# yassine-cherni/mujoco_ros2_simulation

Measured on AMD Instinct MI355X. Metric: env-steps/sec (whole node), 7-DoF arm+lidar scene at 1/2/4/8 MI355X, higher is better.
Workload: dtype f32

## Files before the change

### include/mrs.h

```cpp
#ifndef MRS_H
#define MRS_H

#include "mrs_model.h"

#ifdef __cplusplus
extern "C" {
#endif

typedef struct mrs_model mrs_model;
typedef struct mrs_batch mrs_batch;

enum {
  MRS_OK = 0,
  MRS_ERR_INVALID = -1,
  MRS_ERR_LOAD = -2,
  MRS_ERR_DEVICE = -3,
  MRS_ERR_UNSUPPORTED = -4
};

enum {
  MRS_FIELD_QPOS = 0,
  MRS_FIELD_QVEL = 1,
  MRS_FIELD_CTRL = 2,
  MRS_FIELD_QFRC_APPLIED = 3,
// ... 103 lines not shown
int mrs_batch_get_contact_wrench(mrs_batch* b, double* host, int env0, int n);
enum {
  MRS_DYNOUT_QFRC_BIAS = 0,
  MRS_DYNOUT_MASS_MATRIX = 1,
  MRS_DYNOUT_SITE_JAC = 2,
  MRS_DYNOUT_SITE_POSE = 3,
  MRS_DYNOUT_COUNT = 4
};
#define MRS_MAX_JAC_SITES 16
int mrs_batch_set_jac_sites(mrs_batch* b, const int* site_ids, int n);
int mrs_batch_dyn_dim(const mrs_batch* b, int which);
float* mrs_batch_dyn_device_ptr(mrs_batch* b, int which);
int mrs_batch_get_dyn(mrs_batch* b, int which, double* host, int env0, int n);
int mrs_batch_get_efc(mrs_batch* b, int env, int max, int* type, double* J, double* R, double* aref,
                      double* force);
int mrs_batch_get_field_device(mrs_batch* b, int field, float* d_out, int env0, int n);
int mrs_batch_sync(mrs_batch* b);
double mrs_batch_last_kernel_ms(mrs_batch* b, int kind);
int mrs_batch_set_timing(mrs_batch* b, int mask);
int mrs_debug_phase_cycles(double* out, int n, int reset);
int mrs_debug_batch_layout(const mrs_batch* b, int* out, int n);
int mrs_debug_pairs(const mrs_model* m, int* geom, int max, int* pruned);
int mrs_debug_plan_layout(const mrs_model* m, int n_envs, int cu_count, int max_contacts, int* out, int n);
int mrs_debug_render_plan(const mrs_model* m, int cam, int n_frames, int max_lds, long long* out, int n);
int mrs_debug_ray_filter(const mrs_model* m, unsigned group_mask, int flags, int bodyexclude, int* out, int max);

#ifdef __cplusplus
}
#endif
#endif
```

### mujoco_ros2_simulation_amd/csrc/capi.cc

```cpp
#include <algorithm>
#include <cstring>
#include <memory>
#include <stdexcept>
#include <string>
#include <vector>

#include "../../include/mrs.h"
#include "hip/batch.h"
#include "mjcf/model.h"
#include "hip/rayfilter.h"
#include "hip/start_rows.h"
#include "mjcf/xml.h"

struct mrs_model {
  mrs::Model m;
};
struct mrs_batch {
  mrs::BatchImpl* impl = nullptr;
  const mrs_model* model = nullptr;
};

namespace {

thread_local std::string g_last_error;
// ... 542 lines not shown
  return mrs::batch_layout(b->impl, out, n);
}

int mrs_debug_plan_layout(const mrs_model* m, int n_envs, int cu_count, int max_contacts, int* out, int n) {
  int k = 0;
  const int rc = guarded([&] {
    if (!m || !out || n < 0) throw std::invalid_argument("null model or output");
    if (n_envs < 1) throw std::invalid_argument("n_envs must be positive");
    k = mrs::plan_layout(m->m, n_envs, cu_count, max_contacts, out, n);
  });
  return rc == MRS_OK ? k : rc;
}

int mrs_debug_pairs(const mrs_model* m, int* geom, int max, int* pruned) {
  int k = 0;
  const int rc = guarded([&] {
    if (!m) throw std::invalid_argument("null model");
    if (max < 0 || (max > 0 && !geom)) throw std::invalid_argument("null output or negative capacity");
    k = mrs::walked_pairs(m->m, geom, max, pruned);
  });
  return rc == MRS_OK ? k : rc;
}

int mrs_debug_render_plan(const mrs_model* m, int cam, int n_frames, int max_lds, long long* out, int n) {
  int k = 0;
  const int rc = guarded([&] {
    if (!m || !out || n < 0) throw std::invalid_argument("null model or output");
    if (n_frames < 1) throw std::invalid_argument("n_frames must be positive");
    if (max_lds < 0) throw std::invalid_argument("negative LDS limit");
    k = mrs::render_plan(m->m, cam, n_frames, max_lds, out, n);
  });
  return rc == MRS_OK ? k : rc;
}

int mrs_debug_ray_filter(const mrs_model* m, unsigned group_mask, int flags, int bodyexclude, int* out, int max) {
  int k = 0;
  const int rc = guarded([&] {
    if (!m) throw std::invalid_argument("null model");
    if (max < 0 || (max > 0 && !out)) throw std::invalid_argument("null output or negative capacity");
    mrs::check_ray_filter(m->m, flags, bodyexclude);
    const std::vector<mrs::RayGeom> list =
        mrs::build_ray_filter(m->m, group_mask, (flags & MRS_RAY_NO_STATIC) != 0, bodyexclude);
    k = static_cast<int>(list.size());
    for (int i = 0; i < k && i < max; ++i) out[i] = list[i].id;
  });
  return rc == MRS_OK ? k : rc;
// ... 4 lines not shown
```

### mujoco_ros2_simulation_amd/csrc/hip/batch.h

```cpp
#pragma once

#include <stdexcept>
#include <string>

namespace mrs {

struct Model;
struct BatchImpl;

struct DeviceError : std::runtime_error { using std::runtime_error::runtime_error; };
struct UnsupportedError : std::runtime_error { using std::runtime_error::runtime_error; };

BatchImpl* batch_create(const Model* model, int n_envs, int device, int max_contacts);
void batch_free(BatchImpl* b);
int batch_num_envs(const BatchImpl* b);
int batch_layout(const BatchImpl* b, int* out, int n);
int plan_layout(const Model& m, int n_envs, int cu_count, int max_contacts, int* out, int n);
int walked_pairs(const Model& m, int* geom, int max, int* pruned);
void batch_set_stream(BatchImpl* b, void* stream);
void batch_reset(BatchImpl* b, int key, int env0, int n);
void batch_set_start_states(BatchImpl* b, const double* qpos, const double* qvel, int count);
void batch_set_start_states_device(BatchImpl* b, const float* d_qpos, const float* d_qvel, int count);
int batch_num_start_states(const BatchImpl* b);
void batch_reset_masked_device(BatchImpl* b, const unsigned char* d_mask, const int* d_key, int key);
void batch_reset_masked(BatchImpl* b, const unsigned char* mask, const int* keys, int key);
void batch_set(BatchImpl* b, int field, const double* host, int env0, int n);
void batch_get(BatchImpl* b, int field, double* host, int env0, int n);
void* batch_device_ptr(BatchImpl* b, int field);
void batch_set_act(BatchImpl* b, const double* host, int env0, int n);
void batch_get_act(BatchImpl* b, double* host, int env0, int n);
float* batch_act_device_ptr(BatchImpl* b);
void batch_set_mocap(BatchImpl* b, const double* pos, const double* quat, int env0, int n);
void batch_get_mocap(BatchImpl* b, double* pos, double* quat, int env0, int n);
float* batch_mocap_pos_device_ptr(BatchImpl* b);
float* batch_mocap_quat_device_ptr(BatchImpl* b);
int batch_param_dim(BatchImpl* b, int param);
void batch_set_param(BatchImpl* b, int param, const double* host, int env0, int n);
void batch_get_param(BatchImpl* b, int param, double* host, int env0, int n);
float* batch_param_device_ptr(BatchImpl* b, int param);
int batch_inertial_dim(BatchImpl* b, int which);
void batch_set_inertial(BatchImpl* b, const double* mass, const double* inertia, const double* armature, int env0, int n);
// ... 31 lines not shown
```

### mujoco_ros2_simulation_amd/csrc/hip/batch.hip

```cpp
#include <hip/hip_runtime.h>

#include <algorithm>
#include <cmath>
#include <cstdio>
#include <cstdlib>
#include <cstring>
#include <deque>
#include <initializer_list>
#include <stdexcept>
#include <string>
#include <thread>
#include <type_traits>
#include <utility>
#include <vector>

#include "../../../include/mrs.h"
#include "../mjcf/model.h"
#include "batch.h"
#include "batch_impl.h"
#include "devmodel.h"
#include "devtables.h"
#include "plan.h"
#include "lit.h"
#include "start_rows.h"
// ... 147 lines not shown
  for (int id = 0; id < kArrCount; ++id) {
    const EnvArray a = env_array(b, id);
    if (a.made == EnvArray::ON_USE || (a.made == EnvArray::IF_DIM && a.dim == 0)) continue;
    a.bind(dalloc(b, static_cast<size_t>(b.n) * std::max(1, a.dim) * a.width()));
  }
}

void build_devmodel(BatchImpl& b, int max_con_req, const Overrides& o) {
  const Model& m = *b.model;
  const DevTables T = build_tables(m, max_con_req, o);
  int cus = 0;
  if (hipDeviceGetAttribute(&cus, hipDeviceAttributeMultiprocessorCount, b.device) != hipSuccess) cus = 0;
  const Plan p = choose_plan(m, T, b.n, cus, o);
  void* made[kArrCount];
  for (int id = 0; id < kArrCount; ++id) made[id] = env_array(b, id).ptr;
  b.dm = p.dm;
  for (int id = 0; id < kArrCount; ++id)
    if (made[id]) env_array(b, id).bind(made[id]);
  b.dblock_f = dalloc(b, T.f.size() * sizeof(float));
  b.dblock_i = dalloc(b, T.i.size() * sizeof(int));
  HIP_CHECK(hipMemcpyAsync(b.dblock_f, T.f.data(), T.f.size() * sizeof(float), hipMemcpyHostToDevice, b.stream));
  HIP_CHECK(hipMemcpyAsync(b.dblock_i, T.i.data(), T.i.size() * sizeof(int), hipMemcpyHostToDevice, b.stream));
  T.patch(b.dm, static_cast<const float*>(b.dblock_f), static_cast<const int*>(b.dblock_i));
  b.dm.rf_static = b.dm.rf_mode ? static_cast<float*>(dalloc(b, std::max(1, b.dm.nrf) * sizeof(float))) : nullptr;
  b.group = p.group; b.g16_one_wg = p.g16_one_wg; b.wpb16 = p.wpb16; b.helpers = p.helpers; b.ext = p.ext;
  b.pair_g1 = T.pair_g1; b.pair_g2 = T.pair_g2; b.pair_dim = T.pair_dim; b.pair_mu = T.pair_mu;
  b.pairs_pruned = T.pairs_pruned;
  b.d_dm = static_cast<DevModel*>(dalloc(b, sizeof(DevModel)));
  HIP_CHECK(hipMemcpyAsync(b.d_dm, &b.dm, sizeof(DevModel), hipMemcpyHostToDevice, b.stream));
  HIP_CHECK(hipStreamSynchronize(b.stream));
}

struct RowStage { double* host; std::vector<float> f; std::vector<int> i; };

void rows_to_device(BatchImpl& b, int env0, int n, std::initializer_list<std::pair<EnvArray, const double*>> parts) {
  HIP_CHECK(hipSetDevice(b.device));
  std::deque<RowStage> stage;
  bool queued = false;
  for (const auto& part : parts) {
    const EnvArray& a = part.first;
    const double* host = part.second;
    const size_t cnt = static_cast<size_t>(n) * std::max(0, a.dim);
    if (!host || cnt == 0) continue;
    const void* src = host;
    if (a.type == EnvArray::F32) {
      std::vector<float>& t = stage.emplace_back().f;
      t.resize(cnt);
// ... 207 lines not shown
  return b;
}

void batch_free(BatchImpl* b) {
  if (!b) return;
  (void)hipSetDevice(b->device);
  if (b->stream) (void)hipStreamSynchronize(b->stream);
  if (b->rstream) (void)hipStreamSynchronize(b->rstream);
  for (void* p : b->allocs) (void)hipFree(p);
  if (b->pool_qpos) (void)hipFree(b->pool_qpos);
  if (b->pool_qvel) (void)hipFree(b->pool_qvel);
  render_free(*b);
  for (int k = 0; k < 2; ++k) {
    if (b->ev0[k]) (void)hipEventDestroy(b->ev0[k]);
    if (b->ev1[k]) (void)hipEventDestroy(b->ev1[k]);
  }
  if (b->own_stream) (void)hipStreamDestroy(b->own_stream);
  delete b;
}

int batch_num_envs(const BatchImpl* b) { return b->n; }

int batch_layout(const BatchImpl* b, int* out, int n) {
  int v[21];
  plan_layout_values(b->dm, b->group, b->g16_one_wg, b->wpb16, b->helpers, v);
  v[16] = b->dm.cfrc_contact ? 1 : 0;
  v[17] = b->dm.dyn_mask;
  v[18] = b->dm.solve_fuse;
  v[19] = b->dm.npair;
  v[20] = b->pairs_pruned;
  int k = 0;
  for (; k < n && k < 21; ++k) out[k] = v[k];
  return k;
}

int walked_pairs(const Model& m, int* geom, int max, int* pruned) {
  const DevTables T = build_tables(m, 0, read_overrides());
  const int k = static_cast<int>(T.pair_g1.size());
  for (int q = 0; q < k && q < max; ++q) { geom[2 * q] = T.pair_g1[q]; geom[2 * q + 1] = T.pair_g2[q]; }
  if (pruned) *pruned = T.pairs_pruned;
  return k;
}

int plan_layout(const Model& m, int n_envs, int cu_count, int max_contacts, int* out, int n) {
  const Overrides o = read_overrides();
  const DevTables T = build_tables(m, max_contacts, o);
  const Plan p = choose_plan(m, T, n_envs, cu_count, o);
  int v[kPlanLayoutValues];
  plan_layout_values(p.dm, p.group, p.g16_one_wg, p.wpb16, p.helpers, v);
  int k = 0;
  for (; k < n && k < kPlanLayoutValues; ++k) out[k] = v[k];
  return k;
}

void batch_set_stream(BatchImpl* b, void* stream) {
  b->stream = stream ? static_cast<hipStream_t>(stream) : b->own_stream;
}

void batch_reset(BatchImpl* b, int key, int env0, int n) {
  const Model& m = *b->model;
  check_env_range(*b, env0, n);
  if (key >= m.nkey) throw std::invalid_argument("keyframe index out of range");
  b->ctrl_bound = nullptr;
  if (n == 0) return;
// ... 504 lines not shown
```

### mujoco_ros2_simulation_amd/csrc/hip/devmodel.h

```cpp
#pragma once

#include <cstdint>

#include "../../../include/mrs_model.h"

namespace mrs {

#if !defined(__HIPCC__)
#define __device__
#define __forceinline__ inline
#endif
template <class T>
struct CPtr {
  const T* p;
  CPtr& operator=(const T* q) { p = q; return *this; }
  __device__ __forceinline__ T operator[](int i) const {
#if defined(__HIP_DEVICE_COMPILE__)
    return ((const __attribute__((address_space(4))) T*)p)[i];
#else
    return p[i];
#endif
  }
  __device__ __forceinline__ CPtr operator+(int i) const { return CPtr{p + i}; }
};
// ... 119 lines not shown
  CPtr<float> rfray;
  int rf_sweep, rf_sw_n, rf_sw_full, rf_sw_adr0, rf_sw_plo, rf_sw_phi;
  float rf_sw[16];
  const float* xfrc;
  int na;
  int prm_mask;
  CPtr<float> actdyn;
  int nmocap;
  float *mocap_pos, *mocap_quat;
  const float *prm_gain, *prm_bias, *prm_damp, *prm_fric;
  int npair_explicit;
  const float* prm_inr;
  int inr_dim;
  float* cfrc_contact;
  int dyn_mask, dyn_nsel;
  float* dyn_out[4];
  int dyn_site[16];
  int solve_fuse;
  int nten_spatial, lds_tenJ;
  CPtr<int> tsp_ten, tsp_adr, tsp_num, ten_sp;
  CPtr<float> tsp_seg;
  int nact_site, nact_site_vel;
  CPtr<float> sact;
};
constexpr int kRayBlock = 128;
constexpr int kPrmGain = 1, kPrmBias = 2, kPrmDamp = 4, kPrmFric = 8;
constexpr int kPrmInr = 16;
constexpr int kDynBias = 1, kDynM = 2, kDynJac = 4, kDynPose = 8;

template <int G>
#ifndef MRS_G16_WAVES
#define MRS_G16_WAVES 4
#endif
struct WavesPerBlock { static constexpr int value = G == 64 ? 1 : (G == 16 ? MRS_G16_WAVES : 4); };
inline int envs_per_block(int g, int wpb16 = WavesPerBlock<16>::value) {
  switch (g) {
    case 8: return WavesPerBlock<8>::value * 8;
    case 16: return wpb16 * 4;
    case 32: return WavesPerBlock<32>::value * 2;
    default: return WavesPerBlock<64>::value;
  }
}

struct DevState {
  float *qpos, *qvel, *ctrl, *qfrc_applied, *qacc_ws, *qacc, *qfrc_act, *sensordata;
  double* time;
// ... 17 lines not shown
```

### mujoco_ros2_simulation_amd/csrc/hip/devtables.h

```cpp
#pragma once

#include <algorithm>
#include <array>
#include <cmath>
#include <cstdlib>
#include <cstring>
#include <functional>
#include <stdexcept>
#include <string>
#include <vector>

#include "../../../include/mrs.h"
#include "../mjcf/model.h"
#include "batch.h"
#include "devmodel.h"
#include "renderplan.h"
#include "start_rows.h"

namespace mrs {

struct Overrides {
  int group = 0;
  int g16_wpb = 0;
  bool g16_one_wg = false;
  bool ray_helpers = true;
  bool no_fuse_ih = false;
  bool no_solve_fuse = false;
  bool no_ray_sweep = false;
  bool no_pair_prune = false;
  bool no_static_rays = false;
  bool no_static_frame = false;
  bool kin_twopass = false;
  int sparse_off = 0;
  int diag_skip = 0;
  bool sensors_every_step = false;
  bool no_multiccd = false;
  bool no_bvh = false;
  int bvh_leaf = 4;
  bool bvh_median = false;
  int spread = 0;
};

inline Overrides read_overrides() {
  auto set = [](const char* name) { return std::getenv(name) != nullptr; };
  auto num = [](const char* name, int absent) { const char* e = std::getenv(name); return e ? std::atoi(e) : absent; };
  Overrides o;
  o.group = num("MRS_GROUP", 0);
  o.g16_wpb = num("MRS_G16_WPB", 0);
  o.g16_one_wg = set("MRS_G16_ONE_WG");
  o.ray_helpers = num("MRS_RAY_HELPERS", 1) != 0;
  o.no_fuse_ih = set("MRS_NO_FUSE_IH");
  o.no_solve_fuse = set("MRS_NO_SOLVE_FUSE");
  o.no_ray_sweep = set("MRS_NO_RAY_SWEEP");
  o.no_pair_prune = set("MRS_NO_PAIR_PRUNE");
  o.no_static_rays = set("MRS_NO_STATIC_RAYS");
  o.no_static_frame = set("MRS_NO_STATIC_FRAME");
  o.kin_twopass = set("MRS_KIN_TWOPASS");
  o.sparse_off = num("MRS_SPARSE_OFF", 0) & 15;
  o.diag_skip = num("MRS_DIAG_SKIP", 0);
  o.sensors_every_step = num("MRS_SENSORS_EVERY_STEP", 0) != 0;
  o.no_multiccd = set("MRS_NO_MULTICCD");
  o.no_bvh = set("MRS_NO_BVH");
  o.bvh_leaf = std::max(1, std::min(64, num("MRS_BVH_LEAF", 4)));
  o.bvh_median = set("MRS_BVH_MEDIAN");
  o.spread = std::max(0, std::min(3, num("MRS_SPREAD", 0)));
  return o;
}

constexpr int kRlitHead = 12, kRlitLight = 24, kRlitMat = 12, kRlitTex = 16, kRlitMaxLights = 8;

template <class T>
struct Slot {
  CPtr<T> DevModel::*member;
  size_t off, len;
};
// ... 9 lines not shown
  int pairs_pruned = 0;
  bool convex_pairs = false;
  std::vector<int> rf;
  bool rf_fixed = false;

  void addf(CPtr<float> DevModel::*dst, const std::vector<double>& v) {
    fslot.push_back({dst, f.size(), v.size()});
    for (double x : v) f.push_back(static_cast<float>(x));
    while (f.size() % 4) f.push_back(0);
  }
  void addf(CPtr<float> DevModel::*dst, const std::vector<float>& v) {
    fslot.push_back({dst, f.size(), v.size()});
    f.insert(f.end(), v.begin(), v.end());
    while (f.size() % 4) f.push_back(0);
  }
  void addi(CPtr<int> DevModel::*dst, const std::vector<int>& v) {
    islot.push_back({dst, i.size(), v.size()});
    i.insert(i.end(), v.begin(), v.end());
    while (i.size() % 4) i.push_back(0);
  }
  const float* table(CPtr<float> DevModel::*member) const {
    for (const auto& s : fslot)
      if (s.member == member) return f.data() + s.off;
    throw std::logic_error("table not packed");
  }
  void patch(DevModel& d, const float* fbase, const int* ibase) const {
    for (const auto& s : fslot) (d.*s.member).p = fbase + s.off;
    for (const auto& s : islot) (d.*s.member).p = ibase + s.off;
  }
};

inline float int_bits(int v) { float f; std::memcpy(&f, &v, sizeof f); return f; }
inline int bits_int(float f) { int v; std::memcpy(&v, &f, sizeof v); return v; }

inline void quat_to_mat(const double q[4], double R[9]) {
  R[0] = q[0] * q[0] + q[1] * q[1] - q[2] * q[2] - q[3] * q[3]; R[1] = 2 * (q[1] * q[2] - q[0] * q[3]);
  R[2] = 2 * (q[1] * q[3] + q[0] * q[2]); R[3] = 2 * (q[1] * q[2] + q[0] * q[3]);
  R[4] = q[0] * q[0] - q[1] * q[1] + q[2] * q[2] - q[3] * q[3]; R[5] = 2 * (q[2] * q[3] - q[0] * q[1]);
  R[6] = 2 * (q[1] * q[3] - q[0] * q[2]); R[7] = 2 * (q[2] * q[3] + q[0] * q[1]);
  R[8] = q[0] * q[0] - q[1] * q[1] - q[2] * q[2] + q[3] * q[3];
}

inline std::array<double, 3> site_z_axis(const Model& m, int site) {
  double R[9];
  quat_to_mat(&m.site_quat[4 * site], R);
  const double n = std::sqrt(R[2] * R[2] + R[5] * R[5] + R[8] * R[8]);
// ... 1057 lines not shown
  tree_records(m, trees, bodytab, mpairtab);
  T.addf(&D::bodytab, bodytab);
  T.addf(&D::mpairtab, mpairtab);
  kinematics_records(m, kb, kj, kg);
  T.addf(&D::kinbody, kb);
  T.addf(&D::kinjnt, kj);
  T.addf(&D::kingeom, kg);
  T.addf(&D::sensrec, sensor_records(m, rows, trees));
  T.rf = rows.rf;
  T.rf_fixed = d.nrf > 0;
  for (int s : T.rf) T.rf_fixed = T.rf_fixed && fixed_in_world(m, m.site_bodyid[m.sensor_objid[s]]);
  d.rf_static_frame = T.rf_fixed && !o.no_static_frame ? 1 : 0;
  T.addf(&D::rgeom, ray_geom_records(m, d));
  T.addf(&D::rfblk, ray_block_records(m, T.rf, d));
  T.addf(&D::rfray, ray_records(m, T.rf, d));
  if (d.nten_spatial > 0) {
    T.addi(&D::tsp_ten, ten.sp_ten); T.addi(&D::tsp_adr, ten.sp_adr); T.addi(&D::tsp_num, ten.sp_num);
    T.addi(&D::ten_sp, ten.sp_of); T.addf(&D::tsp_seg, ten.sp_seg);
  }
  if (d.nact_site > 0) T.addf(&D::sact, act.site);
  return T;
}

}
```

### mujoco_ros2_simulation_amd/csrc/hip/step.hip

```cpp
#include <hip/hip_runtime.h>

#include "devmodel.h"
#include "raymesh.h"
#include "rayprim.h"
#include "step_launch.h"
#include "step/base.h"
#include "step/math.h"


namespace mrs {

namespace {

struct Con { float dist, pos[3], nrm[3]; };
typedef __attribute__((address_space(1))) Con gCon;

__device__ __forceinline__ int sphere_sphere(const float p1[3], float r1, const float p2[3], float r2,
                                             float margin, gCon* out, int n) {
  float dv[3] = {p2[0] - p1[0], p2[1] - p1[1], p2[2] - p1[2]};
  float len = sqrtf(dot3(dv, dv));
  float dist = len - r1 - r2;
  if (dist > margin || n >= 4) return n;
  gCon& c = out[n];
  if (len < kMinVal) { c.nrm[0] = 1; c.nrm[1] = c.nrm[2] = 0; }
// ... 7127 lines not shown
template <int G>
__device__ void rk4_final(ENV_PARAMS) {
  ENV_UNPACK;
  const int nq = m.nq, nv = m.nv;
  const float h = m.timestep;
  lfloat* q0 = s + L.rk;
  lfloat* v0 = q0 + (nq > 1 ? nq : 1);
  lfloat *sv = v0 + 2 * nv, *sa = sv + nv;
  #pragma unroll 1
  for (int j = lane; j < nv; j += G) {
    const float acc = s[L.qacc + j];
    sv[j] += (1.0f / 6) * s[L.qvel + j];
    const float dA = sa[j] + (1.0f / 6) * acc;
    s[L.qacc_ws + j] = acc;
    s[L.qvel + j] = v0[j] + h * dA;
  }
  #pragma unroll 1
  for (int i = lane; i < nq; i += G) s[L.qpos + i] = q0[i];
  wsync();
  integrate_pos<G>(m, s, sv, h, lane);
}

template <int G>
#ifndef MRS_G64_WAVES
#define MRS_G64_WAVES 2
#endif
#ifndef MRS_G16_OCC
#define MRS_G16_OCC 2
#endif
struct Occupancy { static constexpr int waves = G == 64 ? MRS_G64_WAVES : (G == 32 ? 4 : (G == 16 ? MRS_G16_OCC : 1)); };

template <int G, bool kForwardOnly, bool kPrimal = false, bool kHelpers = false>
#ifndef MRS_HELPER_OCC
#define MRS_HELPER_OCC 1
#endif
__global__ __launch_bounds__(64 * WavesPerBlock<G>::value, kHelpers ? MRS_HELPER_OCC : Occupancy<G>::waves) void step_kernel(
    const DevModel* __restrict__ mp, DevState st, int n_envs, int n_steps) {
  extern __shared__ __attribute__((aligned(16))) float smem[];
  const int kEnvsPerBlock = G == 16 ? 4 * st.wpb16 : WavesPerBlock<G>::value * 64 / G;
  const DevModel& m = *mp;
  const LdsLayout& L = m.L;
  constexpr bool helpers = G == 16 && !kForwardOnly && kHelpers;
  const bool is_helper = helpers && threadIdx.x >= 64 * st.wpb16;
  const int tid = is_helper ? threadIdx.x - 64 * st.wpb16 : threadIdx.x;
  const int lane = tid & (G - 1), slot = tid / G;
  const int vgroup = blockIdx.x * kEnvsPerBlock + slot;
  const int env = vgroup >> st.spread_shift;
  const bool primary = (vgroup & ((1 << st.spread_shift) - 1)) == 0;
  const bool valid = env < n_envs && primary;
  lfloat* s = (lfloat*)(smem + slot * L.total);
  gfloat* scr = (gfloat*)(st.scratch + (size_t)(valid || st.spread_shift == 0 ? env : st.scr_mirror + vgroup) * m.S.total);
  const size_t e = (size_t)(env < n_envs ? env : n_envs - 1);
  #pragma unroll 1
  for (int i = lane; i < (is_helper ? 0 : m.nq); i += G) s[L.qpos + i] = st.qpos[e * m.nq + i];
  #pragma unroll 1
  for (int i = lane; i < (is_helper ? 0 : m.nv); i += G) {
    s[L.qvel + i] = st.qvel[e * m.nv + i];
    s[L.qfrc_applied + i] = st.qfrc_applied[e * m.nv + i];
    s[L.qacc_ws + i] = st.qacc_ws[e * m.nv + i];
  }
  #pragma unroll 1
  for (int i = lane; i < (is_helper ? 0 : m.nu); i += G) s[L.ctrl + i] = st.ctrl[e * m.nu + i];
  #pragma unroll 1
  for (int i = lane; i < (is_helper ? 0 : m.na); i += G) {
    s[L.act + i] = st.act[e * m.na + i];
    s[L.act + m.na + i] = 0;
  }
  if (m.nmocap > 0) {
    #pragma unroll 1
    for (int i = lane; i < (is_helper ? 0 : 7 * m.nmocap); i += G) {
      const int k = i / 7, c = i - 7 * k;
      s[L.mocap + i] = c < 3 ? m.mocap_pos[(e * m.nmocap + k) * 3 + c] : m.mocap_quat[(e * m.nmocap + k) * 4 + c - 3];
    }
  }
  if ((st.xfrc_applied || (kPrm && m.prm_mask) || m.cfrc_contact || (kDynOut && m.dyn_mask)) && lane == 0 && !is_helper) scr[m.S.xfrc] = __int_as_float(env < n_envs ? env : -1);
  if constexpr (G == 64) {
    #pragma unroll 1
    for (int t = lane; t < m.ntree; t += G) {
      s[L.trees + 4 * t] = __int_as_float(m.tree_dofadr[t]);
      s[L.trees + 4 * t + 1] = __int_as_float(m.tree_dofnum[t]);
      s[L.trees + 4 * t + 2] = __int_as_float(m.tree_Moff[t]);
      s[L.trees + 4 * t + 3] = 0;
    }
    #pragma unroll 1
    for (int j = lane; j < m.nv; j += G) {
      const int bj = m.dof_bodyid[j];
      s[L.dofb + 2 * j] = __int_as_float(bj);
      s[L.dofb + 2 * j + 1] = __int_as_float(m.body_subtree_end[bj]);
    }
  }
  double time = st.time[e];
  gfloat* sensordata = valid ? (gfloat*)(st.sensordata + e * m.nsensordata) : scr + m.S.sens;
  {
    float* shr = smem + m.shr_off;
    #pragma unroll 1
    for (int i = threadIdx.x; i < m.shr_rf; i += blockDim.x) shr[i] = m.rgeom[i];
    #pragma unroll 1
    for (int i = threadIdx.x; i < m.shr_rfst - m.shr_rf; i += blockDim.x) shr[m.shr_rf + i] = m.rfray[8 * (i >> 2) + (i & 3)];
    if (m.rf_mode == 2)
      #pragma unroll 1
      for (int i = threadIdx.x; i < m.nrf; i += blockDim.x) shr[m.shr_rfst + i] = m.rf_static[i];
    #pragma unroll 1
    for (int i = threadIdx.x; i < 17 * m.nrfblk; i += blockDim.x) shr[m.shr_blk + i] = m.rfblk[i];
    #pragma unroll 1
    for (int i = threadIdx.x; i < m.shr_fric - m.shr_sens; i += blockDim.x) shr[m.shr_sens + i] = m.sensrec[i];
    #pragma unroll 1
    for (int i = threadIdx.x; i < 4 * m.nfric; i += blockDim.x) shr[m.shr_fric + i] = m.fricrec[i];
    #pragma unroll 1
    for (int i = threadIdx.x; i < 4 * m.nlim; i += blockDim.x) shr[m.shr_lim + i] = m.limrec[i];
    if constexpr (G < 64) {
      #pragma unroll 1
      for (int i = threadIdx.x; i < 20 * m.nu; i += blockDim.x) shr[m.shr_act + i] = m.actrec[i];
      #pragma unroll 1
      for (int i = threadIdx.x; i < 16 * m.nv; i += blockDim.x) shr[m.shr_dof + i] = m.dofrec[i];
      #pragma unroll 1
      for (int i = threadIdx.x; i < 8 * m.nbody; i += blockDim.x) shr[m.shr_body + i] = m.bodytab[i];
      #pragma unroll 1
      for (int i = threadIdx.x; i < 4 * m.nMpair; i += blockDim.x) shr[m.shr_mpair + i] = m.mpairtab[i];
      #pragma unroll 1
      for (int i = threadIdx.x; i < m.njump * m.nbody; i += blockDim.x) shr[m.shr_jump + i] = __int_as_float(m.jump[i]);
      #pragma unroll 1
      for (int i = threadIdx.x; i < 25 * m.nbody; i += blockDim.x) shr[m.shr_kbody + i] = m.kinbody[i];
      #pragma unroll 1
      for (int i = threadIdx.x; i < 13 * m.njnt; i += blockDim.x) shr[m.shr_kjnt + i] = m.kinjnt[i];
      #pragma unroll 1
      for (int i = threadIdx.x; i < 9 * m.ngeom; i += blockDim.x) shr[m.shr_kgeom + i] = m.kingeom[i];
    }
  }
  if (helpers && threadIdx.x < 4) *helper_flag(m, threadIdx.x) = 0;
  __syncthreads();
  wsync();
  if (is_helper) {
    const int hwave = (__builtin_amdgcn_readfirstlane(threadIdx.x) >> 6) - st.wpb16;
    int timeouts = 0;
    #pragma unroll 1
    for (int step = 0; step < n_steps; ++step) {
      helper_barrier(false);
      int nc = 0, nr = -1;
      if (!(m.diag_skip & 2)) MRS_CALL(G, nc = collision<G>(ENV_ARGS));
      if (helper_rows(m)) {
        if (helper_wait(m, hwave, step + 1)) {
          [[clang::noinline]] nr = dense_rows<G>(ENV_ARGS, nc);
          MRS_CALL(G, dense_impedance<G>(ENV_ARGS, nr));
        } else {
          ++timeouts;
        }
      }
      if (lane == 0) s[L.hcon] = __int_as_float(nc + 65536 * (nr + 1));
      helper_barrier(true);
      if (m.sens_every || step == n_steps - 1) MRS_CALL(G, rays_pass<G>(ENV_ARGS, sensordata));
      if (L.Lh != 0) MRS_CALL(G, integrate_prefactor<G>(ENV_ARGS));
// ... 197 lines not shown
```

### mujoco_ros2_simulation_amd/sim.py

```python
from __future__ import annotations

import ctypes as C
import os
from pathlib import Path

import numpy as np

_PKG = Path(__file__).resolve().parent
LIB_PATH = Path(os.environ["MRS_LIB"]) if os.environ.get("MRS_LIB") else _PKG / "libmrs.so"

GEOM_PLANE, GEOM_HFIELD, GEOM_SPHERE, GEOM_CAPSULE, GEOM_ELLIPSOID, GEOM_CYLINDER, GEOM_BOX, GEOM_MESH = range(8)
JNT_FREE, JNT_BALL, JNT_SLIDE, JNT_HINGE = range(4)
OBJ_BODY, OBJ_JOINT, OBJ_GEOM, OBJ_SITE, OBJ_CAMERA, OBJ_ACTUATOR, OBJ_SENSOR = 1, 3, 5, 6, 7, 19, 20
OBJ_TENDON = 18
SENS_ACCELEROMETER, SENS_GYRO, SENS_FORCE, SENS_TORQUE, SENS_RANGEFINDER = 1, 3, 4, 5, 7
SENS_JOINTPOS, SENS_JOINTVEL, SENS_ACTUATORFRC, SENS_FRAMEPOS, SENS_FRAMEQUAT = 9, 10, 15, 25, 26
SENS_TOUCH, SENS_VELOCIMETER, SENS_FRAMEXAXIS, SENS_FRAMEYAXIS, SENS_FRAMEZAXIS = 0, 2, 27, 28, 29
SENS_FRAMELINVEL, SENS_FRAMEANGVEL, SENS_FRAMELINACC, SENS_SUBTREECOM, SENS_SUBTREELINVEL = 30, 31, 32, 34, 35
SENS_TENDONPOS, SENS_TENDONVEL = 11, 12
BIAS_NONE, BIAS_AFFINE = 0, 1
RESTATE_NEWTON_REFINE, RESTATE_PGS_ELLIPTIC_BLOCK, RESTATE_NO_MPR_POLISH, RESTATE_NO_MULTICCD = 1, 2, 4, 8
(FIELD_QPOS, FIELD_QVEL, FIELD_CTRL, FIELD_QFRC_APPLIED, FIELD_QACC_WARMSTART, FIELD_QACC,
 FIELD_QFRC_ACTUATOR, FIELD_SENSORDATA, FIELD_TIME, FIELD_WARNING, FIELD_NCON, FIELD_SOLVER_NITER,
 FIELD_XFRC_APPLIED) = range(13)
# ... 233 lines not shown
            L.mrs_batch_get_contact_wrench.argtypes = [C.c_void_p, C.c_void_p, C.c_int, C.c_int]
        if hasattr(L, "mrs_batch_get_dyn"):
            L.mrs_batch_set_jac_sites.argtypes = [C.c_void_p, C.c_void_p, C.c_int]
            L.mrs_batch_dyn_dim.argtypes = [C.c_void_p, C.c_int]
            L.mrs_batch_dyn_device_ptr.restype = C.c_void_p
            L.mrs_batch_dyn_device_ptr.argtypes = [C.c_void_p, C.c_int]
            L.mrs_batch_get_dyn.argtypes = [C.c_void_p, C.c_int, C.c_void_p, C.c_int, C.c_int]
        if hasattr(L, "mrs_batch_ray"):
            L.mrs_batch_ray_device.argtypes = [C.c_void_p, C.c_void_p, C.c_void_p, C.c_int, C.c_int, C.c_int, C.c_int,
                                               C.c_uint, C.c_int, C.c_void_p, C.c_void_p]
            L.mrs_batch_ray.argtypes = [C.c_void_p, C.c_void_p, C.c_void_p, C.c_int, C.c_int, C.c_int, C.c_int,
                                        C.c_uint, C.c_int, C.c_void_p, C.c_void_p, C.c_int, C.c_int]
            L.mrs_debug_ray_filter.argtypes = [C.c_void_p, C.c_uint, C.c_int, C.c_int, C.c_void_p, C.c_int]
        L.mrs_batch_get_field_device.argtypes = [C.c_void_p, C.c_int, C.c_void_p, C.c_int, C.c_int]
        L.mrs_batch_last_kernel_ms.restype = C.c_double
        L.mrs_batch_last_kernel_ms.argtypes = [C.c_void_p, C.c_int]
        L.mrs_debug_phase_cycles.argtypes = [C.c_void_p, C.c_int, C.c_int]
        L.mrs_debug_batch_layout.argtypes = [C.c_void_p, C.c_void_p, C.c_int]
        L.mrs_debug_plan_layout.argtypes = [C.c_void_p, C.c_int, C.c_int, C.c_int, C.c_void_p, C.c_int]
        if hasattr(L, "mrs_debug_render_plan"):
            L.mrs_debug_render_plan.argtypes = [C.c_void_p, C.c_int, C.c_int, C.c_int, C.c_void_p, C.c_int]
        if hasattr(L, "mrs_debug_pairs"):
            L.mrs_debug_pairs.argtypes = [C.c_void_p, C.c_void_p, C.c_int, C.c_void_p]
        _lib = L
    return _lib


PHASES = ["kinematics", "com_pos", "make_M", "cholesky", "com_vel", "rne", "smooth_forces", "collision",
          "constraints", "sensors", "integrate", "checks", "sensors.level1", "sensors.setup", "sensors.geoms",
          "constraints.rows", "constraints.records", "constraints.warmstart", "constraints.pgs",
          "collision.narrow", "collision.out", "constraints.delassus", "records.jac", "records.solve",
          "records.rows"]


def phase_cycles(reset: bool = False) -> dict | None:
    out = np.zeros(len(PHASES))
    n = lib().mrs_debug_phase_cycles(out.ctypes.data_as(C.c_void_p), len(PHASES), int(reset))
    if n <= 0:
        return None
    return dict(zip(PHASES, out[:n].tolist()))


def _check(rc: int) -> None:
    if rc != MRS_OK:
        raise MrsError(rc, lib().mrs_last_error().decode())

# ... 84 lines not shown
        return self._h

    def __del__(self):
        if getattr(self, "_h", None) and _lib is not None:
            _lib.mrs_model_free(self._h)
            self._h = None


_FIELD_DIM = {
    FIELD_QPOS: (1, "nq"), FIELD_QVEL: (1, "nv"), FIELD_CTRL: (1, "nu"), FIELD_QFRC_APPLIED: (1, "nv"),
    FIELD_QACC_WARMSTART: (1, "nv"), FIELD_QACC: (1, "nv"), FIELD_QFRC_ACTUATOR: (1, "nv"),
    FIELD_SENSORDATA: (1, "nsensordata"), FIELD_TIME: (1, None), FIELD_WARNING: (4, None), FIELD_NCON: (1, None),
    FIELD_SOLVER_NITER: (1, None), FIELD_XFRC_APPLIED: (6, "nbody"),
}


LAYOUT_KEYS = ["group", "lds_floats", "scratch_floats", "blocked", "pipe_w", "max_efc", "max_con", "ntree",
               "shared_floats", "rf_common", "one_workgroup_per_cu", "waves_per_workgroup", "helper_waves",
               "fused_integrator_factor", "ray_sweep", "sensors_every_step"]
LAYOUT_OUTPUT_KEYS = ["contact_wrench"]
LAYOUT_DYN_KEYS = ["dyn_outputs"]
LAYOUT_SOLVE_KEYS = ["solve_fuse"]
LAYOUT_PAIR_KEYS = ["pairs", "pairs_pruned"]


def plan_layout(model: "Model", n_envs: int, cu_count: int, max_contacts: int = 0) -> dict:
    out = np.zeros(len(LAYOUT_KEYS), dtype=np.int32)
    k = lib().mrs_debug_plan_layout(model.handle, n_envs, cu_count, max_contacts, out.ctypes.data, len(out))
    if k < 0:
        raise MrsError(k, lib().mrs_last_error().decode())
    return dict(zip(LAYOUT_KEYS[:k], out[:k].tolist()))


def walked_pairs(model: "Model") -> tuple[np.ndarray, int]:
    pruned = C.c_int(0)
    k = lib().mrs_debug_pairs(model.handle, None, 0, C.byref(pruned))
    if k < 0:
        raise MrsError(k, lib().mrs_last_error().decode())
    out = np.zeros((k, 2), dtype=np.int32)
    lib().mrs_debug_pairs(model.handle, out.ctypes.data if k else None, k, None)
    return out, pruned.value


RENDER_KERNELS = ["binned", "frame", "tile"]


def render_plan(model: "Model", cam: int, n_frames: int, max_lds: int) -> dict:
    out = np.zeros(7, dtype=np.int64)
    k = lib().mrs_debug_render_plan(model.handle, cam, n_frames, max_lds, out.ctypes.data, len(out))
    if k < 0:
        raise MrsError(k, lib().mrs_last_error().decode())
    v = out.tolist()
    return {"kernel": RENDER_KERNELS[v[0]], "mesh": bool(v[1]), "band_lds": v[2], "chunk": v[3], "per_frame": v[4],
            "grid": (v[5], v[6])}


def ray_filter(model: "Model", group_mask: int = 0, include_static: bool = True, bodyexclude: int = -1) -> np.ndarray:
    out = np.zeros(max(1, model.ngeom), dtype=np.int32)
    k = lib().mrs_debug_ray_filter(model.handle, group_mask, 0 if include_static else RAY_NO_STATIC, bodyexclude,
                                   out.ctypes.data, model.ngeom)
    if k < 0:
        raise MrsError(k, lib().mrs_last_error().decode())
    return out[:k].copy()

# ... 144 lines not shown

    def reset_where(self, mask, keys=None, key: int = -1) -> None:
        mask = np.asarray(mask)
        if mask.shape != (self.n,):
            raise ValueError(f"mask must have shape ({self.n},), not {mask.shape}")
        if mask.dtype not in (np.bool_, np.uint8):
            raise ValueError(f"mask must be bool or uint8, not {mask.dtype}")
        mask = np.ascontiguousarray(mask).view(np.uint8)
        if keys is not None:
            keys = np.asarray(keys)
            if keys.shape != (self.n,):
                raise ValueError(f"keys must have shape ({self.n},), not {keys.shape}")
            if keys.dtype != np.int32:
                raise ValueError(f"keys must be int32, not {keys.dtype}")
            keys = np.ascontiguousarray(keys)
        _check(lib().mrs_batch_reset_masked(self._h, mask.ctypes.data, keys.ctypes.data if keys is not None else None,
                                             key))

    def reset_where_device(self, mask_ptr: int, keys_ptr: int = 0, key: int = -1) -> None:
        _check(lib().mrs_batch_reset_masked_device(self._h, C.c_void_p(mask_ptr) if mask_ptr else None,
                                                    C.c_void_p(keys_ptr) if keys_ptr else None, key))

    def layout(self) -> dict:
        keys = LAYOUT_KEYS + LAYOUT_OUTPUT_KEYS + LAYOUT_DYN_KEYS + LAYOUT_SOLVE_KEYS + LAYOUT_PAIR_KEYS
        out = np.zeros(len(keys), dtype=np.int32)
        k = lib().mrs_debug_batch_layout(self._h, out.ctypes.data, len(keys))
        return dict(zip(keys[:k], out[:k].tolist()))

    def step(self, n_steps: int = 1) -> None:
        _check(lib().mrs_batch_step(self._h, n_steps))

    def forward(self) -> None:
        _check(lib().mrs_batch_forward(self._h))

    def sync(self) -> None:
        _check(lib().mrs_batch_sync(self._h))

    def device_ptr(self, field: int) -> int:
        return lib().mrs_batch_device_ptr(self._h, field)

    def set_ctrl_device(self, ptr: int) -> None:
        _check(lib().mrs_batch_set_ctrl_device(self._h, C.c_void_p(ptr)))

    def bind_ctrl_device(self, ptr: int | None) -> None:
        _check(lib().mrs_batch_bind_ctrl_device(self._h, C.c_void_p(ptr) if ptr else None))

    def set_stream(self, stream_ptr: int | None) -> None:
# ... 137 lines not shown
```

Baseline: 304.5 million.

## Stage shared model tables from one pre-packed contiguous image with vectorized loads

Packs all the per-model tables that each workgroup copies into LDS into a single contiguous device image on the host. At kernel entry they are then staged with batched 16-byte loads from the constant address space, replacing many small strided per-table loops. The first-lane per-env state loads are also hoisted ahead of the table staging so their latency overlaps with it. This adds host-side packing, an extra device allocation and debug APIs, and keeps the old path behind an env override.

```diff
diff --git a/include/mrs.h b/include/mrs.h
--- a/include/mrs.h
+++ b/include/mrs.h
@@ -149,6 +149,9 @@
 int mrs_debug_batch_layout(const mrs_batch* b, int* out, int n);
 int mrs_debug_pairs(const mrs_model* m, int* geom, int max, int* pruned);
 int mrs_debug_plan_layout(const mrs_model* m, int n_envs, int cu_count, int max_contacts, int* out, int n);
+int mrs_debug_table_image(const mrs_model* m, int n_envs, int cu_count, int max_contacts, float* image, int max,
+                          int* offsets, int n_off);
+int mrs_debug_staged_table(const mrs_model* m, int max_contacts, int which, float* out, int max);
 int mrs_debug_render_plan(const mrs_model* m, int cam, int n_frames, int max_lds, long long* out, int n);
 int mrs_debug_ray_filter(const mrs_model* m, unsigned group_mask, int flags, int bodyexclude, int* out, int max);
 
diff --git a/mujoco_ros2_simulation_amd/csrc/capi.cc b/mujoco_ros2_simulation_amd/csrc/capi.cc
--- a/mujoco_ros2_simulation_amd/csrc/capi.cc
+++ b/mujoco_ros2_simulation_amd/csrc/capi.cc
@@ -588,6 +588,29 @@
   return rc == MRS_OK ? k : rc;
 }
 
+int mrs_debug_table_image(const mrs_model* m, int n_envs, int cu_count, int max_contacts, float* image, int max,
+                          int* offsets, int n_off) {
+  int k = 0;
+  const int rc = guarded([&] {
+    if (!m) throw std::invalid_argument("null model");
+    if (n_envs < 1) throw std::invalid_argument("n_envs must be positive");
+    if (max < 0 || (max > 0 && !image) || n_off < 0 || (n_off > 0 && !offsets))
+      throw std::invalid_argument("null output or negative capacity");
+    k = mrs::table_image(m->m, n_envs, cu_count, max_contacts, image, max, offsets, n_off);
+  });
+  return rc == MRS_OK ? k : rc;
+}
+
+int mrs_debug_staged_table(const mrs_model* m, int max_contacts, int which, float* out, int max) {
+  int k = 0;
+  const int rc = guarded([&] {
+    if (!m) throw std::invalid_argument("null model");
+    if (max < 0 || (max > 0 && !out)) throw std::invalid_argument("null output or negative capacity");
+    k = mrs::staged_table(m->m, max_contacts, which, out, max);
+  });
+  return rc == MRS_OK ? k : rc;
+}
+
 int mrs_debug_render_plan(const mrs_model* m, int cam, int n_frames, int max_lds, long long* out, int n) {
   int k = 0;
   const int rc = guarded([&] {
diff --git a/mujoco_ros2_simulation_amd/csrc/hip/batch.h b/mujoco_ros2_simulation_amd/csrc/hip/batch.h
--- a/mujoco_ros2_simulation_amd/csrc/hip/batch.h
+++ b/mujoco_ros2_simulation_amd/csrc/hip/batch.h
@@ -17,6 +17,8 @@
 int batch_layout(const BatchImpl* b, int* out, int n);
 int plan_layout(const Model& m, int n_envs, int cu_count, int max_contacts, int* out, int n);
 int walked_pairs(const Model& m, int* geom, int max, int* pruned);
+int table_image(const Model& m, int n_envs, int cu_count, int max_contacts, float* image, int max, int* offsets, int n_off);
+int staged_table(const Model& m, int max_contacts, int which, float* out, int max);
 void batch_set_stream(BatchImpl* b, void* stream);
 void batch_reset(BatchImpl* b, int key, int env0, int n);
 void batch_set_start_states(BatchImpl* b, const double* qpos, const double* qvel, int count);
diff --git a/mujoco_ros2_simulation_amd/csrc/hip/batch.hip b/mujoco_ros2_simulation_amd/csrc/hip/batch.hip
--- a/mujoco_ros2_simulation_amd/csrc/hip/batch.hip
+++ b/mujoco_ros2_simulation_amd/csrc/hip/batch.hip
@@ -193,7 +193,17 @@
   HIP_CHECK(hipMemcpyAsync(b.dblock_f, T.f.data(), T.f.size() * sizeof(float), hipMemcpyHostToDevice, b.stream));
   HIP_CHECK(hipMemcpyAsync(b.dblock_i, T.i.data(), T.i.size() * sizeof(int), hipMemcpyHostToDevice, b.stream));
   T.patch(b.dm, static_cast<const float*>(b.dblock_f), static_cast<const int*>(b.dblock_i));
-  b.dm.rf_static = b.dm.rf_mode ? static_cast<float*>(dalloc(b, std::max(1, b.dm.nrf) * sizeof(float))) : nullptr;
+  const std::vector<float> image = o.no_table_image ? std::vector<float>() : pack_shared_image(T, b.dm);
+  float* d_image = nullptr;
+  if (!o.no_table_image) {
+    d_image = static_cast<float*>(dalloc(b, image.size() * sizeof(float)));
+    if (!image.empty())
+      HIP_CHECK(hipMemcpyAsync(d_image, image.data(), image.size() * sizeof(float), hipMemcpyHostToDevice, b.stream));
+    b.dm.shr_image = d_image;
+  }
+  b.dm.rf_static = !b.dm.rf_mode ? nullptr
+                   : d_image     ? d_image + b.dm.shr_rfst
+                                 : static_cast<float*>(dalloc(b, std::max(1, b.dm.nrf) * sizeof(float)));
   b.group = p.group; b.g16_one_wg = p.g16_one_wg; b.wpb16 = p.wpb16; b.helpers = p.helpers; b.ext = p.ext;
   b.pair_g1 = T.pair_g1; b.pair_g2 = T.pair_g2; b.pair_dim = T.pair_dim; b.pair_mu = T.pair_mu;
   b.pairs_pruned = T.pairs_pruned;
@@ -447,15 +457,16 @@
 int batch_num_envs(const BatchImpl* b) { return b->n; }
 
 int batch_layout(const BatchImpl* b, int* out, int n) {
-  int v[21];
+  int v[22];
   plan_layout_values(b->dm, b->group, b->g16_one_wg, b->wpb16, b->helpers, v);
   v[16] = b->dm.cfrc_contact ? 1 : 0;
   v[17] = b->dm.dyn_mask;
   v[18] = b->dm.solve_fuse;
   v[19] = b->dm.npair;
   v[20] = b->pairs_pruned;
+  v[21] = b->dm.shr_image.p ? 1 : 0;
   int k = 0;
-  for (; k < n && k < 21; ++k) out[k] = v[k];
+  for (; k < n && k < 22; ++k) out[k] = v[k];
   return k;
 }
 
@@ -465,6 +476,42 @@
   for (int q = 0; q < k && q < max; ++q) { geom[2 * q] = T.pair_g1[q]; geom[2 * q + 1] = T.pair_g2[q]; }
   if (pruned) *pruned = T.pairs_pruned;
   return k;
+}
+
+int table_image(const Model& m, int n_envs, int cu_count, int max_contacts, float* image, int max, int* offsets, int n_off) {
+  const Overrides o = read_overrides();
+  const DevTables T = build_tables(m, max_contacts, o);
+  const Plan p = choose_plan(m, T, n_envs, cu_count, o);
+  const DevModel& d = p.dm;
+  const std::vector<float> img = pack_shared_image(T, d);
+  for (int k = 0; k < max && k < static_cast<int>(img.size()); ++k) image[k] = img[k];
+  const int off[18] = {d.shr_rf, d.shr_rfst, d.shr_blk, d.shr_sens, d.shr_fric, d.shr_lim, d.shr_act, d.shr_dof, d.shr_body,
+                       d.shr_mpair, d.shr_jump, d.shr_kbody, d.shr_kjnt, d.shr_kgeom, d.shr_flag, d.shr_total, d.blocked,
+                       shared_image_floats(d)};
+  for (int k = 0; k < n_off && k < 18; ++k) offsets[k] = off[k];
+  return static_cast<int>(img.size());
+}
+
+int staged_table(const Model& m, int max_contacts, int which, float* out, int max) {
+  using D = DevModel;
+  const DevTables T = build_tables(m, max_contacts, read_overrides());
+  CPtr<float> D::*const ftab[14] = {&D::rgeom, &D::rfray, &D::rfblk, &D::sensrec, &D::fricrec, &D::limrec, &D::actrec,
+                                    &D::dofrec, &D::bodytab, &D::mpairtab, nullptr, &D::kinbody, &D::kinjnt, &D::kingeom};
+  if (which < 0 || which >= 14) throw std::invalid_argument("unknown staged table");
+  if (!ftab[which]) {
+    for (const auto& s : T.islot)
+      if (s.member == &D::jump) {
+        for (size_t k = 0; k < s.len && static_cast<int>(k) < max; ++k) out[k] = int_bits(T.i[s.off + k]);
+        return static_cast<int>(s.len);
+      }
+    throw std::logic_error("table not packed");
+  }
+  for (const auto& s : T.fslot)
+    if (s.member == ftab[which]) {
+      for (size_t k = 0; k < s.len && static_cast<int>(k) < max; ++k) out[k] = T.f[s.off + k];
+      return static_cast<int>(s.len);
+    }
+  throw std::logic_error("table not packed");
 }
 
 int plan_layout(const Model& m, int n_envs, int cu_count, int max_contacts, int* out, int n) {
diff --git a/mujoco_ros2_simulation_amd/csrc/hip/devmodel.h b/mujoco_ros2_simulation_amd/csrc/hip/devmodel.h
--- a/mujoco_ros2_simulation_amd/csrc/hip/devmodel.h
+++ b/mujoco_ros2_simulation_amd/csrc/hip/devmodel.h
@@ -165,6 +165,7 @@
   CPtr<float> tsp_seg;
   int nact_site, nact_site_vel;
   CPtr<float> sact;
+  CPtr<float> shr_image;
 };
 constexpr int kRayBlock = 128;
 constexpr int kPrmGain = 1, kPrmBias = 2, kPrmDamp = 4, kPrmFric = 8;
diff --git a/mujoco_ros2_simulation_amd/csrc/hip/devtables.h b/mujoco_ros2_simulation_amd/csrc/hip/devtables.h
--- a/mujoco_ros2_simulation_amd/csrc/hip/devtables.h
+++ b/mujoco_ros2_simulation_amd/csrc/hip/devtables.h
@@ -26,6 +26,7 @@
   bool ray_helpers = true;
   bool no_fuse_ih = false;
   bool no_solve_fuse = false;
+  bool no_table_image = false;
   bool no_ray_sweep = false;
   bool no_pair_prune = false;
   bool no_static_rays = false;
@@ -51,6 +52,7 @@
   o.ray_helpers = num("MRS_RAY_HELPERS", 1) != 0;
   o.no_fuse_ih = set("MRS_NO_FUSE_IH");
   o.no_solve_fuse = set("MRS_NO_SOLVE_FUSE");
+  o.no_table_image = set("MRS_NO_TABLE_IMAGE");
   o.no_ray_sweep = set("MRS_NO_RAY_SWEEP");
   o.no_pair_prune = set("MRS_NO_PAIR_PRUNE");
   o.no_static_rays = set("MRS_NO_STATIC_RAYS");
@@ -106,6 +108,11 @@
   const float* table(CPtr<float> DevModel::*member) const {
     for (const auto& s : fslot)
       if (s.member == member) return f.data() + s.off;
+    throw std::logic_error("table not packed");
+  }
+  const int* itable(CPtr<int> DevModel::*member) const {
+    for (const auto& s : islot)
+      if (s.member == member) return i.data() + s.off;
     throw std::logic_error("table not packed");
   }
   void patch(DevModel& d, const float* fbase, const int* ibase) const {
@@ -1209,4 +1216,35 @@
   return T;
 }
 
-}
+inline int shared_image_floats(const DevModel& d) { return d.blocked ? d.shr_act : d.shr_flag; }
+
+inline std::vector<float> pack_shared_image(const DevTables& T, const DevModel& d) {
+  using D = DevModel;
+  const int n = shared_image_floats(d);
+  std::vector<float> img(static_cast<size_t>((n + 3) & ~3), 0.0f);
+  auto put = [&](int off, int end, const float* src) {
+    for (int k = off; k < end && k < n; ++k) img[k] = src[k - off];
+  };
+  put(0, d.shr_rf, T.table(&D::rgeom));
+  const float* rfray = T.table(&D::rfray);
+  for (int k = d.shr_rf; k < d.shr_rfst; ++k) {
+    const int q = k - d.shr_rf;
+    img[k] = rfray[8 * (q >> 2) + (q & 3)];
+  }
+  put(d.shr_blk, d.shr_sens, T.table(&D::rfblk));
+  put(d.shr_sens, d.shr_fric, T.table(&D::sensrec));
+  put(d.shr_fric, d.shr_lim, T.table(&D::fricrec));
+  put(d.shr_lim, d.shr_act, T.table(&D::limrec));
+  put(d.shr_act, d.shr_dof, T.table(&D::actrec));
+  put(d.shr_dof, d.shr_body, T.table(&D::dofrec));
+  put(d.shr_body, d.shr_mpair, T.table(&D::bodytab));
+  put(d.shr_mpair, d.shr_jump, T.table(&D::mpairtab));
+  const int* jump = T.itable(&D::jump);
+  for (int k = d.shr_jump; k < d.shr_kbody && k < n; ++k) img[k] = int_bits(jump[k - d.shr_jump]);
+  put(d.shr_kbody, d.shr_kjnt, T.table(&D::kinbody));
+  put(d.shr_kjnt, d.shr_kgeom, T.table(&D::kinjnt));
+  put(d.shr_kgeom, d.shr_flag, T.table(&D::kingeom));
+  return img;
+}
+
+}
diff --git a/mujoco_ros2_simulation_amd/csrc/hip/step.hip b/mujoco_ros2_simulation_amd/csrc/hip/step.hip
--- a/mujoco_ros2_simulation_amd/csrc/hip/step.hip
+++ b/mujoco_ros2_simulation_amd/csrc/hip/step.hip
@@ -7173,6 +7173,70 @@
 }
 
 template <int G>
+__device__ void stage_tables(const DevModel& m, float* shr) {
+  #pragma unroll 1
+  for (int i = threadIdx.x; i < m.shr_rf; i += blockDim.x) shr[i] = m.rgeom[i];
+  #pragma unroll 1
+  for (int i = threadIdx.x; i < m.shr_rfst - m.shr_rf; i += blockDim.x) shr[m.shr_rf + i] = m.rfray[8 * (i >> 2) + (i & 3)];
+  if (m.rf_mode == 2)
+    #pragma unroll 1
+    for (int i = threadIdx.x; i < m.nrf; i += blockDim.x) shr[m.shr_rfst + i] = m.rf_static[i];
+  #pragma unroll 1
+  for (int i = threadIdx.x; i < 17 * m.nrfblk; i += blockDim.x) shr[m.shr_blk + i] = m.rfblk[i];
+  #pragma unroll 1
+  for (int i = threadIdx.x; i < m.shr_fric - m.shr_sens; i += blockDim.x) shr[m.shr_sens + i] = m.sensrec[i];
+  #pragma unroll 1
+  for (int i = threadIdx.x; i < 4 * m.nfric; i += blockDim.x) shr[m.shr_fric + i] = m.fricrec[i];
+  #pragma unroll 1
+  for (int i = threadIdx.x; i < 4 * m.nlim; i += blockDim.x) shr[m.shr_lim + i] = m.limrec[i];
+  if constexpr (G < 64) {
+    #pragma unroll 1
+    for (int i = threadIdx.x; i < 20 * m.nu; i += blockDim.x) shr[m.shr_act + i] = m.actrec[i];
+    #pragma unroll 1
+    for (int i = threadIdx.x; i < 16 * m.nv; i += blockDim.x) shr[m.shr_dof + i] = m.dofrec[i];
+    #pragma unroll 1
+    for (int i = threadIdx.x; i < 8 * m.nbody; i += blockDim.x) shr[m.shr_body + i] = m.bodytab[i];
+    #pragma unroll 1
+    for (int i = threadIdx.x; i < 4 * m.nMpair; i += blockDim.x) shr[m.shr_mpair + i] = m.mpairtab[i];
+    #pragma unroll 1
+    for (int i = threadIdx.x; i < m.njump * m.nbody; i += blockDim.x) shr[m.shr_jump + i] = __int_as_float(m.jump[i]);
+    #pragma unroll 1
+    for (int i = threadIdx.x; i < 25 * m.nbody; i += blockDim.x) shr[m.shr_kbody + i] = m.kinbody[i];
+    #pragma unroll 1
+    for (int i = threadIdx.x; i < 13 * m.njnt; i += blockDim.x) shr[m.shr_kjnt + i] = m.kinjnt[i];
+    #pragma unroll 1
+    for (int i = threadIdx.x; i < 9 * m.ngeom; i += blockDim.x) shr[m.shr_kgeom + i] = m.kingeom[i];
+  }
+}
+
+#ifndef MRS_IMAGE_DEPTH
+#define MRS_IMAGE_DEPTH 4
+#endif
+constexpr int kImageDepth = MRS_IMAGE_DEPTH;
+typedef float f32x4 __attribute__((ext_vector_type(4)));
+__device__ __forceinline__ void stage_table_image(const DevModel& m, float* shr, int n) {
+  const __attribute__((address_space(4))) f32x4* img = (const __attribute__((address_space(4))) f32x4*)m.shr_image.p;
+  const int nvec = (n + 3) >> 2, stride = blockDim.x;
+  #pragma unroll 1
+  for (int base = threadIdx.x; base < nvec; base += kImageDepth * stride) {
+    f32x4 v[kImageDepth];
+    #pragma unroll
+    for (int k = 0; k < kImageDepth; ++k) v[k] = img[min(base + k * stride, nvec - 1)];
+    #pragma unroll
+    for (int k = 0; k < kImageDepth; ++k) {
+      const int i = base + k * stride;
+      if (4 * i + 4 <= n) {
+        *(f32x4*)(shr + 4 * i) = v[k];
+      } else if (i < nvec) {
+        const float w[4] = {v[k].x, v[k].y, v[k].z, v[k].w};
+        for (int c = 0; c < 4; ++c)
+          if (4 * i + c < n) shr[4 * i + c] = w[c];
+      }
+    }
+  }
+}
+
+template <int G>
 #ifndef MRS_G64_WAVES
 #define MRS_G64_WAVES 2
 #endif
@@ -7202,18 +7266,42 @@
   lfloat* s = (lfloat*)(smem + slot * L.total);
   gfloat* scr = (gfloat*)(st.scratch + (size_t)(valid || st.spread_shift == 0 ? env : st.scr_mirror + vgroup) * m.S.total);
   const size_t e = (size_t)(env < n_envs ? env : n_envs - 1);
-  #pragma unroll 1
-  for (int i = lane; i < (is_helper ? 0 : m.nq); i += G) s[L.qpos + i] = st.qpos[e * m.nq + i];
-  #pragma unroll 1
-  for (int i = lane; i < (is_helper ? 0 : m.nv); i += G) {
+  const int nq_l = is_helper ? 0 : m.nq, nv_l = is_helper ? 0 : m.nv, nu_l = is_helper ? 0 : m.nu, na_l = is_helper ? 0 : m.na;
+  float q0 = 0, v0 = 0, fa0 = 0, ws0 = 0, c0 = 0, a0 = 0;
+  if (lane < nq_l) q0 = st.qpos[e * m.nq + lane];
+  if (lane < nv_l) {
+    v0 = st.qvel[e * m.nv + lane];
+    fa0 = st.qfrc_applied[e * m.nv + lane];
+    ws0 = st.qacc_ws[e * m.nv + lane];
+  }
+  if (lane < nu_l) c0 = st.ctrl[e * m.nu + lane];
+  if (lane < na_l) a0 = st.act[e * m.na + lane];
+  double time = st.time[e];
+  if (m.shr_image.p) stage_table_image(m, smem + m.shr_off, G == 64 ? m.shr_act : m.shr_flag);
+  else { [[clang::noinline]] stage_tables<G>(m, smem + m.shr_off); }
+  if (lane < nq_l) s[L.qpos + lane] = q0;
+  if (lane < nv_l) {
+    s[L.qvel + lane] = v0;
+    s[L.qfrc_applied + lane] = fa0;
+    s[L.qacc_ws + lane] = ws0;
+  }
+  if (lane < nu_l) s[L.ctrl + lane] = c0;
+  if (lane < na_l) {
+    s[L.act + lane] = a0;
+    s[L.act + m.na + lane] = 0;
+  }
+  #pragma unroll 1
+  for (int i = lane + G; i < nq_l; i += G) s[L.qpos + i] = st.qpos[e * m.nq + i];
+  #pragma unroll 1
+  for (int i = lane + G; i < nv_l; i += G) {
     s[L.qvel + i] = st.qvel[e * m.nv + i];
     s[L.qfrc_applied + i] = st.qfrc_applied[e * m.nv + i];
     s[L.qacc_ws + i] = st.qacc_ws[e * m.nv + i];
   }
   #pragma unroll 1
-  for (int i = lane; i < (is_helper ? 0 : m.nu); i += G) s[L.ctrl + i] = st.ctrl[e * m.nu + i];
-  #pragma unroll 1
-  for (int i = lane; i < (is_helper ? 0 : m.na); i += G) {
+  for (int i = lane + G; i < nu_l; i += G) s[L.ctrl + i] = st.ctrl[e * m.nu + i];
+  #pragma unroll 1
+  for (int i = lane + G; i < na_l; i += G) {
     s[L.act + i] = st.act[e * m.na + i];
     s[L.act + m.na + i] = 0;
   }
@@ -7240,44 +7328,7 @@
       s[L.dofb + 2 * j + 1] = __int_as_float(m.body_subtree_end[bj]);
     }
   }
-  double time = st.time[e];
   gfloat* sensordata = valid ? (gfloat*)(st.sensordata + e * m.nsensordata) : scr + m.S.sens;
-  {
-    float* shr = smem + m.shr_off;
-    #pragma unroll 1
-    for (int i = threadIdx.x; i < m.shr_rf; i += blockDim.x) shr[i] = m.rgeom[i];
-    #pragma unroll 1
-    for (int i = threadIdx.x; i < m.shr_rfst - m.shr_rf; i += blockDim.x) shr[m.shr_rf + i] = m.rfray[8 * (i >> 2) + (i & 3)];
-    if (m.rf_mode == 2)
-      #pragma unroll 1
-      for (int i = threadIdx.x; i < m.nrf; i += blockDim.x) shr[m.shr_rfst + i] = m.rf_static[i];
-    #pragma unroll 1
-    for (int i = threadIdx.x; i < 17 * m.nrfblk; i += blockDim.x) shr[m.shr_blk + i] = m.rfblk[i];
-    #pragma unroll 1
-    for (int i = threadIdx.x; i < m.shr_fric - m.shr_sens; i += blockDim.x) shr[m.shr_sens + i] = m.sensrec[i];
-    #pragma unroll 1
-    for (int i = threadIdx.x; i < 4 * m.nfric; i += blockDim.x) shr[m.shr_fric + i] = m.fricrec[i];
-    #pragma unroll 1
-    for (int i = threadIdx.x; i < 4 * m.nlim; i += blockDim.x) shr[m.shr_lim + i] = m.limrec[i];
-    if constexpr (G < 64) {
-      #pragma unroll 1
-      for (int i = threadIdx.x; i < 20 * m.nu; i += blockDim.x) shr[m.shr_act + i] = m.actrec[i];
-      #pragma unroll 1
-      for (int i = threadIdx.x; i < 16 * m.nv; i += blockDim.x) shr[m.shr_dof + i] = m.dofrec[i];
-      #pragma unroll 1
-      for (int i = threadIdx.x; i < 8 * m.nbody; i += blockDim.x) shr[m.shr_body + i] = m.bodytab[i];
-      #pragma unroll 1
-      for (int i = threadIdx.x; i < 4 * m.nMpair; i += blockDim.x) shr[m.shr_mpair + i] = m.mpairtab[i];
-      #pragma unroll 1
-      for (int i = threadIdx.x; i < m.njump * m.nbody; i += blockDim.x) shr[m.shr_jump + i] = __int_as_float(m.jump[i]);
-      #pragma unroll 1
-      for (int i = threadIdx.x; i < 25 * m.nbody; i += blockDim.x) shr[m.shr_kbody + i] = m.kinbody[i];
-      #pragma unroll 1
-      for (int i = threadIdx.x; i < 13 * m.njnt; i += blockDim.x) shr[m.shr_kjnt + i] = m.kinjnt[i];
-      #pragma unroll 1
-      for (int i = threadIdx.x; i < 9 * m.ngeom; i += blockDim.x) shr[m.shr_kgeom + i] = m.kingeom[i];
-    }
-  }
   if (helpers && threadIdx.x < 4) *helper_flag(m, threadIdx.x) = 0;
   __syncthreads();
   wsync();
diff --git a/mujoco_ros2_simulation_amd/sim.py b/mujoco_ros2_simulation_amd/sim.py
--- a/mujoco_ros2_simulation_amd/sim.py
+++ b/mujoco_ros2_simulation_amd/sim.py
@@ -279,6 +279,9 @@
             L.mrs_debug_render_plan.argtypes = [C.c_void_p, C.c_int, C.c_int, C.c_int, C.c_void_p, C.c_int]
         if hasattr(L, "mrs_debug_pairs"):
             L.mrs_debug_pairs.argtypes = [C.c_void_p, C.c_void_p, C.c_int, C.c_void_p]
+        if hasattr(L, "mrs_debug_table_image"):
+            L.mrs_debug_table_image.argtypes = [C.c_void_p, C.c_int, C.c_int, C.c_int, C.c_void_p, C.c_int, C.c_void_p, C.c_int]
+            L.mrs_debug_staged_table.argtypes = [C.c_void_p, C.c_int, C.c_int, C.c_void_p, C.c_int]
         _lib = L
     return _lib
 
@@ -409,6 +412,7 @@
 LAYOUT_DYN_KEYS = ["dyn_outputs"]
 LAYOUT_SOLVE_KEYS = ["solve_fuse"]
 LAYOUT_PAIR_KEYS = ["pairs", "pairs_pruned"]
+LAYOUT_IMAGE_KEYS = ["table_image"]
 
 
 def plan_layout(model: "Model", n_envs: int, cu_count: int, max_contacts: int = 0) -> dict:
@@ -427,6 +431,32 @@
     out = np.zeros((k, 2), dtype=np.int32)
     lib().mrs_debug_pairs(model.handle, out.ctypes.data if k else None, k, None)
     return out, pruned.value
+
+
+IMAGE_TABLES = ["rgeom", "rfray", "rf_static", "rfblk", "sensrec", "fricrec", "limrec", "actrec", "dofrec", "bodytab",
+                "mpairtab", "jump", "kinbody", "kinjnt", "kingeom"]
+STAGED_TABLE_IDS = {name: k for k, name in enumerate(t for t in IMAGE_TABLES if t != "rf_static")}
+
+
+def table_image(model: "Model", n_envs: int, cu_count: int, max_contacts: int = 0) -> dict:
+    off = np.zeros(18, dtype=np.int32)
+    k = lib().mrs_debug_table_image(model.handle, n_envs, cu_count, max_contacts, None, 0, off.ctypes.data, len(off))
+    if k < 0:
+        raise MrsError(k, lib().mrs_last_error().decode())
+    img = np.zeros(k, dtype=np.float32)
+    lib().mrs_debug_table_image(model.handle, n_envs, cu_count, max_contacts, img.ctypes.data if k else None, k, None, 0)
+    offsets = dict(zip(IMAGE_TABLES + ["end", "shared_floats"], [0] + off[:16].tolist()))
+    return {"image": img, "offsets": offsets, "blocked": int(off[16]), "copied": int(off[17])}
+
+
+def staged_table(model: "Model", name: str, max_contacts: int = 0) -> np.ndarray:
+    which = STAGED_TABLE_IDS[name]
+    k = lib().mrs_debug_staged_table(model.handle, max_contacts, which, None, 0)
+    if k < 0:
+        raise MrsError(k, lib().mrs_last_error().decode())
+    out = np.zeros(k, dtype=np.float32)
+    lib().mrs_debug_staged_table(model.handle, max_contacts, which, out.ctypes.data if k else None, k)
+    return out
 
 
 RENDER_KERNELS = ["binned", "frame", "tile"]
@@ -617,7 +647,8 @@
                                                     C.c_void_p(keys_ptr) if keys_ptr else None, key))
 
     def layout(self) -> dict:
-        keys = LAYOUT_KEYS + LAYOUT_OUTPUT_KEYS + LAYOUT_DYN_KEYS + LAYOUT_SOLVE_KEYS + LAYOUT_PAIR_KEYS
+        keys = (LAYOUT_KEYS + LAYOUT_OUTPUT_KEYS + LAYOUT_DYN_KEYS + LAYOUT_SOLVE_KEYS + LAYOUT_PAIR_KEYS +
+                LAYOUT_IMAGE_KEYS)
         out = np.zeros(len(keys), dtype=np.int32)
         k = lib().mrs_debug_batch_layout(self._h, out.ctypes.data, len(keys))
         return dict(zip(keys[:k], out[:k].tolist()))
```

Result: faster. 309.1 million, median of 6 (+1.5%).
